# georgeliu233/STrajNet

Hardware: AMD Instinct MI355X
Metric: scenes/sec (fwd+bwd, 256x256 grids) (higher is better)
Workload: dtype bf16; 1 GPU; STrajNet cfg-256 train step (fwd+OGMFlow_loss+bwd+Nadam), batch 8/GPU, 8 waypoints, obs+occ+flow heads, fg_msa+fg, random-init weights; global_batch=8, grid=256x256x11, parallelism=dp1, hipgraph=True, concurrent_branch_streams=True, optimizer_in_step=True, settle_steps=40

## Files before the change

### include/strajnet_hip.h

```cpp
#ifndef STRAJNET_HIP_H
#define STRAJNET_HIP_H
#include <hip/hip_runtime_api.h>
#ifdef __cplusplus
extern "C" {
#endif

enum stj_status { STJ_OK = 0, STJ_EINVAL = -1, STJ_ELAUNCH = -2, STJ_EUNSUPPORTED = -3 };
enum stj_dtype { STJ_F32 = 0, STJ_BF16 = 1, STJ_F16 = 2 };
enum stj_act { STJ_ACT_NONE = 0, STJ_ACT_GELU = 1, STJ_ACT_ELU = 2 };
enum stj_unary { STJ_U_GELU = 1, STJ_U_ELU = 2, STJ_U_TANH_SCALE = 3 };

const char* stj_last_error(void);
int stj_abi_version(void);

int stj_gemm(const void* A, const void* B, void* C, const float* bias, const void* res, float* colsum,
             int M, int N, int K, int nb1, int nb2,
             long long sAb1, long long sAb2, long long sAm, long long sAk,
             long long sBb1, long long sBb2, long long sBk, long long sBn,
             long long sCb1, long long sCb2, long long ldc,
             long long sBias1, long long sBias2, long long sRes1, long long sRes2, long long ldres,
             int act, float alpha, int dtype, int c_f32, int accumulate, int splitk,
             int nkb, long long sAkb, long long sBkb, void* group, hipStream_t stream);
long long stj_gemm_group_workspace_bytes(void);
int stj_gemm_group_begin(void* group);
// ... 174 lines not shown
                       int Wi, int Cin, int Cout, int dtype, hipStream_t stream);
int stj_elu_res_bwd(const void* dy, const void* dy2, const void* y, const void* r, void* dpre, void* gsum, long long n, int dtype,
                    hipStream_t stream);
int stj_skip_junction_bwd(const void* dy1, const void* dy2, const void* y, const void* r1, const void* r2, void* dpre, void* dr1,
                          void* dr2, long long n, int dtype, hipStream_t stream);
int stj_upconv_dgrad(const void* dP, const void* Wd, void* dX, const void* Xelu, int F, int Hi, int Wi, int Cin, int Cout,
                     int dtype, hipStream_t stream);
int stj_upconv_wgrad(const void* X, const void* dP, float* dWeff, float* dbias, int db_parts, int F, int Hi, int Wi, int Cin,
                     int Cout, int wg_budget, int dtype, hipStream_t stream);
int stj_outconv_fwd(const void* X, const float* W, const float* bias, float* Y, int F, int Hh, int Ww, int C, int Tn,
                    long long y_bstride, long long y_tstride, long long y_pstride, int dtype, hipStream_t stream);
int stj_outconv_pair_fwd(const void* X0, const void* X1, const float* W0, const float* W1, const float* bias0, const float* bias1,
                         float* Y, int B, int Tn, int H, int W, int C, int t_major, int dtype, hipStream_t stream);
int stj_upconv_fwd_head(const void* X, const void* Wf, const float* bias, const float* Whead, void* Z, int F, int Hi, int Wi, int Cin,
                        int Cout, int dtype, hipStream_t stream);
int stj_outconv_pair_gather(const void* Z0, const void* Z1, const float* bias0, const float* bias1, float* Y, int B, int Tn, int H, int W,
                            int t_major, int dtype, hipStream_t stream);
int stj_quantize_waypoints(const float* Y, uint8_t* Q, int B, int Tn, int H, int W, hipStream_t stream);
int stj_outconv_pair_gather_q(const void* Z0, const void* Z1, const float* bias0, const float* bias1, uint8_t* Q, int B, int Tn, int H,
                              int W, int t_major, int dtype, hipStream_t stream);
int stj_compress_sizes(int B, int Tn, int H, int W, long long* work_bytes, long long* out_capacity);
int stj_compress_waypoints(const uint8_t* Q, void* work, uint8_t* out, uint32_t* offsets, int B, int Tn, int H, int W, hipStream_t stream);
int stj_outconv_bwd(const void* X, const float* W, const float* dY, void* dX, float* dW, float* db, int F, int Hh, int Ww,
                    int C, int Tn, long long y_bstride, long long y_tstride, long long y_pstride, int elu_in, void* ws,
                    long long ws_bytes, int dtype, hipStream_t stream);
long long stj_outconv_bwd_workspace_bytes(void);
int stj_im2col_patch(const float* src, void* dst, int B, int H, int W, int Cin, long long pix_stride, int ch_stride,
                     int dtype, hipStream_t stream);
int stj_patch_embed_supported(int Cin, int Cout, int dtype);
int stj_patch_embed_fwd(const float* src, const void* w, const float* bias, const float* gamma, const float* beta, const void* add,
                        const float* gamma2, const float* beta2, void* cols, void* pre, void* x2, void* y, float* mean, float* rstd,
                        float* mean2, float* rstd2, int B, int H, int W, int Cin, long long pix_stride, int ch_stride, int Cout,
                        float eps, int dtype, hipStream_t stream);
int stj_im2col3(const void* x, void* cols, int N, int H, int W, int G, int Cg, int dtype, hipStream_t stream);
int stj_col2im3(const void* dcols, void* dx, int N, int H, int W, int G, int Cg, int dtype, hipStream_t stream);

int stj_loss_auc_gate(const float* gt_obs, const float* gt_occ, const float* gt_flow, const float* origin,
                      int* hist, float* gate, float* auc_out, int B, int H, int W, hipStream_t stream);
int stj_loss_fwd(const float* logits, const float* gt_obs, const float* gt_occ, const float* gt_flow, const float* origin,
                 const float* gate, float* sums, float* loss, float* coef, int B, int H, int W, float ogm_w, float occ_w,
                 float flow_origin_w, float replica, int flags, hipStream_t stream);
int stj_loss_bwd(const float* logits, const float* gt_obs, const float* gt_occ, const float* gt_flow, const float* origin,
                 const float* coef, const float* upstream, float* dlogits, int B, int H, int W, int flags, hipStream_t stream);
int stj_loss_coef(const float* gt_flow, const float* gate, int* cnt, float* coef, int B, int H, int W, float ogm_w, float occ_w,
                  float flow_origin_w, float replica, int flags, hipStream_t stream);
int stj_loss_finalize(const float* sums, const float* gate, float* loss, float* coef_out, int B, int H, int W, float ogm_w,
                      float occ_w, float flow_origin_w, float replica, int flags, hipStream_t stream);
int stj_loss_gate_coef(const float* gt_obs, const float* gt_occ, const float* gt_flow, const float* origin, int* hist, float* gate,
                       float* auc_out, float* coef, int B, int H, int W, float ogm_w, float occ_w, float flow_origin_w,
                       float replica, int flags, hipStream_t stream);
int stj_loss_fwd_bwd(const float* logits, const float* gt_obs, const float* gt_occ, const float* gt_flow, const float* origin,
                     const float* gate, const float* coef_in, float* sums, float* loss, float* coef_out, float* dlogits,
                     int B, int H, int W, float ogm_w, float occ_w, float flow_origin_w, float replica, int flags, hipStream_t stream);

int stj_decode_raw(const void* src, int kind, float* dst, long long n_outer, int H, int W, int C, int y0, int x0, int Ho,
                   int Wo, float scale, hipStream_t stream);

int stj_unpack_bits(const uint32_t* bits, float* dst, long long n_total, hipStream_t stream);
int stj_unpack_sparse(const uint32_t* mask, const uint32_t* offs, const uint32_t* val_base, const float* vals, long long n_vals,
                      float* dst, int B, long long n, hipStream_t stream);

int stj_agent_prep(const float* obs, const float* occ, int n_obs, int n_occ, int B, int Tn, void* x5, void* v3, int* vt, int* cmi,
                   void* cmf, int dtype, hipStream_t stream);
int stj_agent_mix_fwd(const void* enc, const void* embed, const void* cm, void* concat, void* qin, int B, int A, int C, int dtype,
                      hipStream_t stream);
int stj_agent_mix_bwd(const void* dconcat, const void* dqin, const void* cm, void* denc, void* dembed, int B, int A, int C, int dtype,
// ... 35 lines not shown
```

### strajnet_amd/build.py

```python
import os
import subprocess
import sys
from concurrent.futures import ThreadPoolExecutor

HERE = os.path.dirname(os.path.abspath(__file__))
CSRC = os.path.join(HERE, 'csrc')
OUT = os.path.join(HERE, 'libstrajnet_hip.so')
HEADER = os.path.join(os.path.dirname(HERE), 'include', 'strajnet_hip.h')
SOURCES = ['util.hip', 'gemm.hip', 'wgrad_sk.hip', 'norm.hip', 'patch_embed.hip', 'swin_attn.hip', 'swin_fused.hip', 'xattn_fused.hip', 'fgattn.hip', 'agent_fused.hip', 'fgoff_fused.hip', 'attn.hip', 'conv.hip', 'conv_ws.hip', 'conv_ps.hip', 'loss.hip', 'eval.hip', 'quantize.hip', 'deflate.hip', 'unpack.hip', 'rng.hip']
FLAGS = ['--offload-arch=gfx950', '-O3', '-std=c++17', '-fPIC', '-munsafe-fp-atomics', '-Wno-unused-result', '-Wno-unused-value',
         '-ffp-contract=fast']


def _hipcc():
    for c in (os.environ.get('HIPCC'), '/opt/rocm/bin/hipcc', 'hipcc'):
        if c and (os.path.sep not in c or os.path.exists(c)):
            return c
    raise RuntimeError('hipcc not found')


def _stale(target, deps):
    if not os.path.exists(target):
        return True
    t = os.path.getmtime(target)
    return any(os.path.getmtime(d) > t for d in deps)


def build(force=False, verbose=True):
    hipcc = _hipcc()
    hdrs = [HEADER] + [os.path.join(CSRC, f) for f in os.listdir(CSRC) if f.endswith('.h')]
    objs, jobs = [], []
    os.makedirs(os.path.join(HERE, 'build'), exist_ok=True)
    for s in SOURCES:
        src = os.path.join(CSRC, s)
        obj = os.path.join(HERE, 'build', s.replace('.hip', '.o'))
        objs.append(obj)
        if force or _stale(obj, [src] + hdrs):
            jobs.append([hipcc] + FLAGS + ['-c', src, '-o', obj])

    def run(cmd):
        r = subprocess.run(cmd, capture_output=True, text=True)
        return cmd, r
# ... 17 lines not shown
```

### strajnet_amd/modules.py

```python
import math
import os
from collections import OrderedDict

import numpy as np
import torch

from . import ops
from .ops import Param, ACT_NONE, ACT_ELU


def _param_spec(cfg, hb, fg_msa, fg):
    C, ws, heads, depths = cfg['embed_dim'], cfg['window_size'], cfg['num_heads'], cfg['depths']
    sp = OrderedDict()

    def add(name, shape, init):
        assert name not in sp
        sp[name] = (tuple(shape), init)

    def dense(n, i, o, bias=True):
        add(n + '/kernel', (i, o), 'glorot')
        if bias:
            add(n + '/bias', (o,), 'zeros')

    def conv(n, kh, kw, i, o, bias=True):
# ... 153 lines not shown
        self._zstride = offs['cross_attn_obs1/norm1/gamma'] - offs['cross_attn_obs0/norm1/gamma']
        for n in spec:
            if n.startswith('cross_attn_obs0/'):
                for z in range(1, 8):
                    assert offs[n.replace('obs0', f'obs{z}')] - offs[n] == z * self._zstride
        self._flat = torch.zeros(off, dtype=torch.float32, device=self.device)
        self._goff8 = (off + ops._ZeroArena.ALIGN - 1) // ops._ZeroArena.ALIGN * ops._ZeroArena.ALIGN
        self._gbuf = torch.zeros(self._goff8 + ops._ZeroArena.FLOATS, dtype=torch.float32, device=self.device)
        self._gflat = self._gbuf[:off]
        self._cflat = self._flat if dtype == torch.float32 else torch.zeros(off, dtype=dtype, device=self.device)
        gen = torch.Generator().manual_seed(seed)
        dpr = np.linspace(0.0, 0.1, sum(cfg['depths']))
        self.drop_path_rate = {}
        for i, d in enumerate(cfg['depths']):
            for j in range(d):
                self.drop_path_rate[f'layers{i}/blocks{j}'] = float(dpr[sum(cfg['depths'][:i]) + j])
        for j in range(cfg['depths'][0]):
            self.drop_path_rate[f'flow_layers0/blocks{j}'] = float(dpr[j])
        self._seg_onehot = {}
        self.dropctx = ops.DropCtx(self.device, seed if dropout_seed is None else dropout_seed)
        self._arena = ops._ZeroArena()
        self._arena.adopt(self._gbuf[self._goff8:])
        self._dctx = None
        self._side = ops.role_stream(self.device, 'side') if (self.device.type == 'cuda' and os.environ.get('STJ_NO_SIDE_STREAM') != '1') else None
        self._side2 = ops.role_stream(self.device, 'side2') if (self._side is not None and os.environ.get('STJ_NO_SIDE_STREAM') != '2') else None
        self._streams = (self._side, self._side2)
        self.serial = False
        self.taps = None
        self.fused_mlp = self.fused_attn = os.environ.get('STJ_FUSED_SWIN', '1') != '0'
        self.fused_attn_dims = (96, 192, 384)
        self.fused_mlp_dims = (96, 192, 384)
        self.fused_xattn = True
        self.fused_stem = True
        self.agent_override = None
        self._quantize_heads = False
        self.mid_forward_hook = None
        self.fused_fgattn = True
        self.fused_agent = True
        self.fused_agent_int = True
        self.fused_quantize = True
        self.fused_fgoff = True
        self._agent_pack = None
        self._agent_pack_event = None
        self._agent_pack_stale = True
        self._fgoff_pack = None
        self._fgoff_pack_event = None
        self._fgoff_pack_stale = True
        self._xattn_pack = None
        self.params = OrderedDict()
        for n, (s, kind) in spec.items():
            k = int(np.prod(s))
            sl = slice(offs[n], offs[n] + k)
            self._flat[sl] = _init_tensor(s, kind, gen).reshape(-1).to(self.device)
            master = self._flat[sl].view(s).requires_grad_(True)
            grad = self._gflat[sl].view(s)
            master.grad = grad
            self.params[n] = Param(n, s, master, self._cflat[sl].view(s), grad)
        def wants_parts(n):
            leaf = n.rsplit('/', 1)[-1]
            if n.startswith('cross_attn_obs'):
                return False
            return leaf in ('gamma', 'beta', 'relative_position_bias_table') or (leaf == 'bias' and '/upconv' in n)
        names = [n for n in spec if wants_parts(n)]
        P = self.PARTS
        self._parts = torch.zeros(P * sum(int(np.prod(spec[n][0])) for n in names), dtype=torch.float32, device=self.device)
        idx, o = [], 0
# ... 120 lines not shown
        qkv = self._dense(h, pre + '/attn/qkv')
        a = ops.win_attn(qkv, self._p(pre + '/attn/relative_position_bias_table'), B, res, heads, shift)

        def mlp_fused(x):
            return ops.swin_mlp(x, self._p(pre + '/norm2/gamma'), self._p(pre + '/norm2/beta'), self._p(pre + '/mlp/fc1/kernel'),
                                self._p(pre + '/mlp/fc1/bias'), self._p(pre + '/mlp/fc2/kernel'), self._p(pre + '/mlp/fc2/bias'), 1e-5,
                                self._dctx, pre + '/drop_path_mlp', dpr, rows_per_sample=res * res)
        if dpr == 0.0:
            x = self._dense(a, pre + '/attn/proj', res=x)
            if fused_mlp:
                return mlp_fused(x)
            h, x = self._ln_skip(x, pre + '/norm2', 1e-5)
            h = ops.gelu(self._dense(h, pre + '/mlp/fc1'))
            return self._dense(h, pre + '/mlp/fc2', res=x)
        a = self._dense(a, pre + '/attn/proj').view(B, -1)
        x = ops.dropout(a, dpr, self._dctx, pre + '/drop_path_attn', res=x.view(B, -1), per_sample=True).view(x.shape)
        if fused_mlp:
            return mlp_fused(x)
        h, x = self._ln_skip(x, pre + '/norm2', 1e-5)
        h = ops.gelu(self._dense(h, pre + '/mlp/fc1'))
        h = self._dense(h, pre + '/mlp/fc2').view(B, -1)
        return ops.dropout(h, dpr, self._dctx, pre + '/drop_path_mlp', res=x.view(B, -1), per_sample=True).view(x.shape)

    def _tap(self, name, t):
        if self.taps is not None:
            self.taps[name] = t.detach().float().clone()

    def _basic_layer(self, x, pre, B, res, depth, heads, downsample, add=None):
        for i in range(depth):
            x = self._swin_block(x, f'{pre}/blocks{i}', B, res, heads, 0 if i % 2 == 0 else 4)
            self._tap(f'{pre}/block{i}', x)
        if not downsample:
            return x, x
        m = self._ln(x, pre + '/downsample/norm', 1e-5, gather_res=res)
        if callable(add):
            add = add()
        return self._dense(m, pre + '/downsample/reduction', bias=False, res=add), x

    def _patch_embed(self, src, name, Cin, ch_stride, pix_stride, add=None, norm2=None):
        B, H = src.shape[0], src.shape[1]
        pw = self._p(name + '/proj/kernel')
        if self.fused_stem and ops.patch_embed_ok(Cin, pw.c.shape[-1], self.dtype):
            y = ops.patch_embed(src, pw, self._p(name + '/proj/bias'), self._p(name + '/norm/gamma'), self._p(name + '/norm/beta'),
                                Cin, ch_stride, pix_stride, self.dtype, 1e-5, add,
                                self._p(norm2 + '/gamma') if norm2 else None, self._p(norm2 + '/beta') if norm2 else None)
            return y.view(B, (H // 4) ** 2, -1)
        cols = ops.patch_im2col(src, Cin, ch_stride, pix_stride, self.dtype)
        y = self._dense(cols, name + '/proj')
        y = self._ln(y, name + '/norm', 1e-5, res=add.view(y.shape) if add is not None else None)
        if norm2:
            y = self._ln(y, norm2, 1e-5)
        return y.view(B, (H // 4) ** 2, -1)

    def _encoder(self, ogm, map_img, flow, hook=None):
        B = ogm.shape[0]
        C, P = self.stage_dim[0], self.P
        depths, heads = self.cfg['depths'], self.cfg['num_heads']
        def flow_branch():
            fl = self._patch_embed(flow, 'patch_embed_flow', 2, 1, 2, norm2='flow_norm')
            return self._basic_layer(fl, 'flow_layers0', B, P, depths[0], heads[0], True)
        side = self._side2
        if side is not None:
            main = torch.cuda.current_stream(self.device)
            side.wait_stream(main)
            with torch.cuda.stream(side):
                flow_x, flow_res = flow_branch()
# ... 441 lines not shown
```

### strajnet_amd/ops.py

```python
import contextlib
import ctypes

import os
import threading

import torch

from . import prof
from ._lib import call as _raw_call, ENUMS as _ENUMS


def call(name, *args):
    if prof.ACTIVE is None:
        return _raw_call(name, *args)
    prof.record(name, args, lambda: _raw_call(name, *args))


GROUP_GEMMS = os.environ.get('STJ_GEMM_GROUP', '1') != '0'
WS_KERNELS = os.environ.get('STJ_NO_WS') != '1'
class _GroupState(threading.local):
    def __init__(self):
        self.h = [None, None]
        self.depth = [0]

# ... 1770 lines not shown
        cols, pre, x2, mean, rstd, mean2, rstd2 = ctx.saved_tensors
        gw, pbias, pg, pb, pg2, pb2 = ctx.p
        M, N = pre.shape
        K = cols.shape[1]
        dy = dy.contiguous().view(M, N)
        if pg2 is not None and LN_CHAIN and _ln_chain_ok(N, dy.dtype):
            dpre = torch.empty_like(pre)
            d2 = torch.empty_like(pre) if ctx.has_add else None
            (g2, b2, n2, s2), (g1, b1, n1, s1) = _ln_grad_targets(pg2, pb2), _ln_grad_targets(pg, pb)
            call('stj_layernorm_bwd_chain', _p(dy), _p(x2), _p(pg2.master), _p(mean2), _p(rstd2), _p(pre), _p(pg.master), _p(mean), _p(rstd),
                 _p(d2), _p(dpre), _p(g2), _p(b2), _p(g1), _p(b1), M, N, n2, s2, n1, s1, _dt(pre), _st())
            dadd = d2.view(ctx.add_shape) if ctx.has_add else None
        else:
            if pg2 is not None:
                dy = _ln_bwd_plain(dy, x2, mean2, rstd2, pg2, pb2, M, N)
            dadd = dy.view(ctx.add_shape) if ctx.has_add else None
            dpre = _ln_bwd_plain(dy, pre, mean, rstd, pg, pb, M, N)
        gemm(cols, dpre, gw, K, N, M, (0, 0, 1, K), (0, 0, N, 1), (0, 0, N), _dt(cols), c_f32=1, accumulate=1, splitk=0,
             colsum=pbias.grad)
        return (None,) * 7 + (dadd,) + (None,) * 4


def patch_embed_ok(Cin, Cout, dtype):
    from ._lib import lib
    return bool(lib().stj_patch_embed_supported(Cin, Cout, DTYPE_CODE[dtype]))


def patch_embed(src, pw, pbias, pg, pb, Cin, ch_stride, pix_stride, dtype, eps=1e-5, add=None, pg2=None, pb2=None):
    N = pw.c.shape[-1]
    return _PatchEmbed.apply(src, pw.master, pw.c.view(-1, N), pw.grad.view(-1, N), pbias, pg, pb, add, pg2, pb2,
                             (Cin, ch_stride, pix_stride, eps, torch.is_grad_enabled()), dtype)


def patch_im2col(src, Cin, ch_stride, pix_stride, dtype):
    _req_cuda(src)
    src = src.contiguous()
    B, H, W = src.shape[0], src.shape[1], src.shape[2]
    out = torch.empty((B * (H // 4) * (W // 4), 16 * Cin), dtype=dtype, device=src.device)
    call('stj_im2col_patch', _p(src), _p(out), B, H, W, Cin, pix_stride, ch_stride, DTYPE_CODE[dtype], _st())
    return out


class _GroupedConv3(torch.autograd.Function):
    @staticmethod
    def forward(ctx, x, w_master, b_master, pw, pb, G):
        _req_cuda(x)
        x = x.contiguous()
        N, H, W, C = x.shape
        Cg = C // G
        K = 9 * Cg
        Co = pw.c.shape[-1]
        cog = Co // G
        dt = _dt(x)
        M = N * H * W
        cols = torch.empty((M, G, K), dtype=x.dtype, device=x.device)
        call('stj_im2col3', _p(x), _p(cols), N, H, W, G, Cg, dt, _st())
        y = torch.empty((N, H, W, Co), dtype=x.dtype, device=x.device)
        gemm(cols, pw.c, y, M, cog, K, (0, K, G * K, 1), (0, cog, Co, 1), (0, cog, Co), dt, bias=pb.master, sBias=(0, cog), nb=(1, G))
        ctx.pw, ctx.pb, ctx.geo = pw, pb, (N, H, W, G, Cg, K, Co, cog, M)
        ctx.save_for_backward(cols)
        return y

    @staticmethod
    def backward(ctx, dy):
        (cols,) = ctx.saved_tensors
        N, H, W, G, Cg, K, Co, cog, M = ctx.geo
# ... 423 lines not shown
```

### strajnet_amd/prof.py

```python
import torch

ACTIVE = None
COST = {}


def enable():
    global ACTIVE
    ACTIVE = {}


def disable():
    global ACTIVE
    p, ACTIVE = ACTIVE, None
    return p


def _es(dt):
    return 4 if dt == 0 else 2


def _gemm(a):
    (M, N, K, nb1, nb2) = a[6:11]
    sAb1, sAb2, sAm, sAk, sBb1, sBb2, sBk, sBn = a[11:19]
    act, alpha, dt, c_f32, acc, splitk, nkb = a[27], a[28], a[29], a[30], a[31], a[32], a[33]
# ... 126 lines not shown


def _elem(fam, n_idx, dt_idx, tensors, f32=False):
    def f(a):
        n = a[n_idx]
        es = 4 if f32 else _es(a[dt_idx])
        return f'{fam}[{n}]', fam, 0.0, 0.0, tensors * es * n
    return f


def _loss(fam, tens):
    def f(a):
        B, H, W = (a[9], a[10], a[11]) if fam == 'loss_fwd' else ((a[11], a[12], a[13]) if fam == 'loss_fwd_bwd' else (a[8], a[9], a[10]))
        by = 4.0 * B * H * W * (32 * tens + 8 * 5)
        return f'{fam}[B{B} {H}x{W}]', fam, 0.0, 0.0, by
    return f


def _eval(a):
    B, H, W = a[11], a[12], a[13]
    return f'eval_fwd[B{B} {H}x{W}]', 'eval_fwd', 0.0, 0.0, 4.0 * B * H * W * (32 + 8 * 5)


def _patch_embed(a):
    B, H, W, Cin, pix, Cout, dt = a[16], a[17], a[18], a[19], a[20], a[22], a[24]
    es = _es(dt)
    M = B * (H // 4) * (W // 4)
    nz = lambda i: bool(getattr(a[i], 'value', None))
    by = 4.0 * B * H * W * pix + es * M * Cout * (1 + nz(5) + nz(9) + nz(10)) + es * M * 16 * Cin * nz(8)
    fl = 2.0 * M * 16 * Cin * Cout
    return f'patch_embed[{H}x{W},{Cin}->{Cout},B{B}]', 'patch_embed_fwd', fl, fl, by


def _ln_chain(a):
    rows, C, dt = a[15], a[16], a[21]
    return f'ln_bwd_chain[{rows}x{C}]', 'layernorm_bwd', 0.0, 0.0, _es(dt) * rows * C * (4 + bool(getattr(a[9], 'value', None)))


MODELS = {
    'stj_gemm': _gemm,
    'stj_patch_embed_fwd': _patch_embed, 'stj_layernorm_bwd_chain': _ln_chain,
    'stj_upconv_fwd': _upconv('fwd'), 'stj_upconv_fwd_head': _upconv_head, 'stj_outconv_pair_gather': _pair_gather, 'stj_outconv_pair_gather_q': _pair_gather_q, 'stj_quantize_waypoints': _quantize, 'stj_compress_waypoints': _compress, 'stj_upconv_fwd_res': _upconv_res, 'stj_elu_res_bwd': _elu_res, 'stj_upconv_dgrad': _upconv('dgrad'), 'stj_upconv_wgrad': _upconv('wgrad'),
    'stj_outconv_fwd': _outconv('fwd'), 'stj_outconv_pair_fwd': _outconv_pair, 'stj_outconv_bwd': _outconv('bwd'),
    'stj_layernorm_fwd': _ln('fwd'), 'stj_layernorm_bwd': _ln('bwd'), 'stj_layernorm_res_fwd': _ln('res_fwd'),
    'stj_win_attn_fwd': _win('fwd'), 'stj_win_attn_bwd': _win('bwd'),
    'stj_unary_fwd': _elem('unary_fwd', 2, 5, 2), 'stj_unary_bwd': _elem('unary_bwd', 3, 6, 3),
    'stj_dropout': _elem('dropout', 3, 8, 2),
    'stj_loss_fwd': _loss('loss_fwd', 1), 'stj_loss_bwd': _loss('loss_bwd', 2), 'stj_loss_fwd_bwd': _loss('loss_fwd_bwd', 2),
    'stj_eval_fwd': _eval,
    'stj_nadam_step': _elem('nadam', 4, 0, 7, f32=True),
}
EXTRA_MODELS = {}


def record(name, args, launch):
    m = MODELS.get(name) or EXTRA_MODELS.get(name)
    if m is not None:
        try:
            key, fam, fa, fe, by = m(args)
        except Exception:
            key, fam, fa, fe, by = name, name.replace('stj_', ''), 0.0, 0.0, 0.0
    else:
        key, fam, fa, fe, by = name, name.replace('stj_', ''), 0.0, 0.0, 0.0
    st = torch.cuda.current_stream()
    e0, e1 = torch.cuda.Event(enable_timing=True), torch.cuda.Event(enable_timing=True)
    e0.record(st)
    launch()
    e1.record(st)
    COST[key] = (fam, fa, fe, by)
    ACTIVE.setdefault(key, []).append((e0, e1))


def summarize(events, steps):
    keys = {}
# ... 15 lines not shown
```

Baseline: 1415 scenes/s.

## Fuse Swin patch-merge gather, LayerNorm and reduction GEMM into one kernel

Adds a patch-merge forward kernel that gathers the 2x2 neighbourhood, applies LayerNorm in registers and runs the reduction matmul from LDS with MFMA, adding the optional residual in the epilogue. A matching backward kernel computes the dgrad GEMM, the LayerNorm backward, the skip-gradient add and the dgamma/dbeta partials, then scatters dx back into the original layout. The goal is to avoid the separate gathered LayerNorm output round trip and several launches at the stage-1/2 downsamples. The weight-grad GEMM stays separate, and the normalized activations are still stored for it when grad is on.

```diff
diff --git a/include/strajnet_hip.h b/include/strajnet_hip.h
--- a/include/strajnet_hip.h
+++ b/include/strajnet_hip.h
@@ -230,6 +230,12 @@
                         const float* gamma2, const float* beta2, void* cols, void* pre, void* x2, void* y, float* mean, float* rstd,
                         float* mean2, float* rstd2, int B, int H, int W, int Cin, long long pix_stride, int ch_stride, int Cout,
                         float eps, int dtype, hipStream_t stream);
+int stj_patch_merge_supported(int C0, int dtype);
+int stj_patch_merge_fwd(const void* x, const float* gamma, const float* beta, const void* w, const void* add, void* y, void* m,
+                        float* mean, float* rstd, int B, int res, int C0, float eps, int dtype, hipStream_t stream);
+int stj_patch_merge_bwd(const void* dy, const void* w, const void* x, const float* gamma, const float* mean, const float* rstd,
+                        const void* dskip, void* dx, float* dgamma, float* dbeta, int B, int res, int C0, int nparts,
+                        long long part_stride, int dtype, hipStream_t stream);
 int stj_im2col3(const void* x, void* cols, int N, int H, int W, int G, int Cg, int dtype, hipStream_t stream);
 int stj_col2im3(const void* dcols, void* dx, int N, int H, int W, int G, int Cg, int dtype, hipStream_t stream);
 
diff --git a/strajnet_amd/build.py b/strajnet_amd/build.py
--- a/strajnet_amd/build.py
+++ b/strajnet_amd/build.py
@@ -7,7 +7,7 @@
 CSRC = os.path.join(HERE, 'csrc')
 OUT = os.path.join(HERE, 'libstrajnet_hip.so')
 HEADER = os.path.join(os.path.dirname(HERE), 'include', 'strajnet_hip.h')
-SOURCES = ['util.hip', 'gemm.hip', 'wgrad_sk.hip', 'norm.hip', 'patch_embed.hip', 'swin_attn.hip', 'swin_fused.hip', 'xattn_fused.hip', 'fgattn.hip', 'agent_fused.hip', 'fgoff_fused.hip', 'attn.hip', 'conv.hip', 'conv_ws.hip', 'conv_ps.hip', 'loss.hip', 'eval.hip', 'quantize.hip', 'deflate.hip', 'unpack.hip', 'rng.hip']
+SOURCES = ['util.hip', 'gemm.hip', 'wgrad_sk.hip', 'norm.hip', 'patch_embed.hip', 'patch_merge.hip', 'swin_attn.hip', 'swin_fused.hip', 'xattn_fused.hip', 'fgattn.hip', 'agent_fused.hip', 'fgoff_fused.hip', 'attn.hip', 'conv.hip', 'conv_ws.hip', 'conv_ps.hip', 'loss.hip', 'eval.hip', 'quantize.hip', 'deflate.hip', 'unpack.hip', 'rng.hip']
 FLAGS = ['--offload-arch=gfx950', '-O3', '-std=c++17', '-fPIC', '-munsafe-fp-atomics', '-Wno-unused-result', '-Wno-unused-value',
          '-ffp-contract=fast']
 
diff --git a/strajnet_amd/csrc/patch_merge.hip b/strajnet_amd/csrc/patch_merge.hip
--- /dev/null
+++ b/strajnet_amd/csrc/patch_merge.hip
@@ -0,0 +1,434 @@
+#include "common.h"
+
+namespace pm {
+
+constexpr int RB = 32;
+constexpr int VN = 8;
+typedef __attribute__((ext_vector_type(4))) uint32_t u32x4;
+
+template <int C0>
+__device__ __forceinline__ size_t src_off(unsigned row, int c, int res) {
+  const unsigned half = (unsigned)res >> 1;
+  const unsigned j = row % half, t = row / half, i = t % half, b = t / half;
+  const int q = c / C0, cc = c - q * C0;
+  return (((size_t)b * res + 2 * i + (q & 1)) * res + 2 * j + (q >> 1)) * C0 + cc;
+}
+template <typename T> __device__ __forceinline__ void unpack8(const uint4& u, float* v) {
+  unpack2<T>(u.x, v[0], v[1]); unpack2<T>(u.y, v[2], v[3]); unpack2<T>(u.z, v[4], v[5]); unpack2<T>(u.w, v[6], v[7]);
+}
+template <typename T> __device__ __forceinline__ uint4 pack8(const float* v) {
+  return make_uint4(pack2<T>(v[0], v[1]), pack2<T>(v[2], v[3]), pack2<T>(v[4], v[5]), pack2<T>(v[6], v[7]));
+}
+
+template <typename T, int WN, int CPR, int N>
+__device__ __forceinline__ void fwd_load_w(u32x4 (&wv)[WN], const T* w, int tid) {
+#pragma unroll
+  for (int j = 0; j < WN; ++j) {
+    const int p = tid + 256 * j, k = p / CPR, c = (p % CPR) * VN;
+    wv[j] = *reinterpret_cast<const u32x4*>(w + (size_t)k * N + c);
+  }
+}
+
+template <typename T, int WN, int CPR, int LDW>
+__device__ __forceinline__ void fwd_stage_w(T* Ws, const u32x4 (&wv)[WN], int tid) {
+  __syncthreads();
+#pragma unroll
+  for (int j = 0; j < WN; ++j) {
+    const int p = tid + 256 * j, k = p / CPR, c = (p % CPR) * VN;
+    *reinterpret_cast<u32x4*>(Ws + k * LDW + c) = wv[j];
+  }
+  __syncthreads();
+}
+template <typename T, int NF, int KC, int LDA, int LDW>
+__device__ __forceinline__ void fwd_mma_chunk(const T* As, const T* Ws, int k0, int rh, int ch, int lane, f32x4 (&acc)[NF]) {
+#pragma unroll
+  for (int kk = 0; kk < KC; kk += 32) {
+    const typename Mma<T>::Frag tok = Mma<T>::load(As, LDA, 16 * rh, k0 + kk, lane);
+#pragma unroll
+    for (int n = 0; n < NF; ++n) acc[n] = Mma<T>::mma(Mma<T>::load_tr(Ws, LDW, (ch * NF + n) * 16, kk, lane), tok, acc[n]);
+  }
+}
+
+struct FwdArgs {
+  const void* x; const float* gamma; const float* beta; const void* w; const void* add;
+  void* y; void* m; float* mean; float* rstd;
+  long long rows; int res; float eps;
+};
+
+template <typename T, int C0, int NF>
+struct FwdGeo {
+  static constexpr int K = 4 * C0, N = 2 * C0, NS = 32 * NF;
+  static constexpr int KC = 12288 / NS;
+  static constexpr int LDA = K + LdsPad<T>::P;
+  static constexpr int LDW = NS + 16;
+  static constexpr size_t lds_bytes = (size_t)(RB * LDA + KC * LDW) * sizeof(T);
+  static_assert(K % KC == 0 && N % NS == 0 && KC % 32 == 0, "whole chunks and slices");
+};
+
+template <typename T, int C0, int NF>
+__global__ __launch_bounds__(256) void patch_merge_fwd_kernel(FwdArgs a) {
+  typedef FwdGeo<T, C0, NF> G;
+  constexpr int K = G::K, N = G::N, NS = G::NS, KC = G::KC, LDA = G::LDA, LDW = G::LDW;
+  constexpr int CPR = NS / VN, WN = KC * CPR / 256;
+  constexpr int NCHK = (K / VN + 63) / 64, RPW = RB / 4;
+  static_assert(KC * CPR % 256 == 0, "whole pieces per thread");
+  extern __shared__ __attribute__((aligned(16))) unsigned char smem[];
+  T* As = reinterpret_cast<T*>(smem);
+  T* Ws = As + RB * LDA;
+  const int tid = threadIdx.x, lane = tid & 63, wave = tid >> 6;
+  const long long m0 = (long long)blockIdx.x * RB;
+  const int n0 = blockIdx.y * NS;
+  const T* w = reinterpret_cast<const T*>(a.w) + n0;
+
+  constexpr int NCH = K / KC;
+  u32x4 wa[WN], wb[WN];
+  fwd_load_w<T, WN, CPR, N>(wa, w, tid);
+  if (NCH > 1) fwd_load_w<T, WN, CPR, N>(wb, w + (size_t)KC * N, tid);
+
+  {
+    const T* x = reinterpret_cast<const T*>(a.x);
+    uint4 raw[RPW][NCHK];
+#pragma unroll
+    for (int u = 0; u < RPW; ++u) {
+      const long long row = min(m0 + wave * RPW + u, a.rows - 1);
+#pragma unroll
+      for (int k = 0; k < NCHK; ++k) {
+        const int c = min((lane + 64 * k) * VN, K - VN);
+        raw[u][k] = *reinterpret_cast<const uint4*>(x + src_off<C0>((unsigned)row, c, a.res));
+      }
+    }
+    float gam[NCHK][VN], bet[NCHK][VN];
+#pragma unroll
+    for (int k = 0; k < NCHK; ++k) {
+      const int c = min((lane + 64 * k) * VN, K - VN);
+#pragma unroll
+      for (int e = 0; e < VN; e += 4) {
+        const float4 gv = *reinterpret_cast<const float4*>(a.gamma + c + e), bv = *reinterpret_cast<const float4*>(a.beta + c + e);
+        gam[k][e] = gv.x; gam[k][e + 1] = gv.y; gam[k][e + 2] = gv.z; gam[k][e + 3] = gv.w;
+        bet[k][e] = bv.x; bet[k][e + 1] = bv.y; bet[k][e + 2] = bv.z; bet[k][e + 3] = bv.w;
+      }
+    }
+    constexpr float invC = 1.f / K;
+#pragma unroll
+    for (int u = 0; u < RPW; ++u) {
+      const int r = wave * RPW + u;
+      const bool ok = m0 + r < a.rows;
+      float v[NCHK][VN];
+      float s = 0.f;
+#pragma unroll
+      for (int k = 0; k < NCHK; ++k) {
+        const bool in = (lane + 64 * k) * VN < K;
+        unpack8<T>(raw[u][k], v[k]);
+#pragma unroll
+        for (int e = 0; e < VN; ++e) { v[k][e] = in ? v[k][e] : 0.f; s += v[k][e]; }
+      }
+      const float mu = wave_sum(s) * invC;
+      float q = 0.f;
+#pragma unroll
+      for (int k = 0; k < NCHK; ++k) {
+        const bool in = (lane + 64 * k) * VN < K;
+#pragma unroll
+        for (int e = 0; e < VN; ++e) { const float d = in ? v[k][e] - mu : 0.f; q += d * d; }
+      }
+      const float rs = rsqrtf(wave_sum(q) * invC + a.eps);
+#pragma unroll
+      for (int k = 0; k < NCHK; ++k) {
+        const int c = (lane + 64 * k) * VN;
+        if (c >= K) continue;
+        float o[VN];
+#pragma unroll
+        for (int e = 0; e < VN; ++e) o[e] = ok ? (v[k][e] - mu) * rs * gam[k][e] + bet[k][e] : 0.f;
+        const uint4 pk = pack8<T>(o);
+        *reinterpret_cast<uint4*>(As + r * LDA + c) = pk;
+        if (a.m && ok && blockIdx.y == 0) *reinterpret_cast<uint4*>(reinterpret_cast<T*>(a.m) + (m0 + r) * K + c) = pk;
+      }
+      if (a.mean && ok && blockIdx.y == 0 && lane == 0) { a.mean[m0 + r] = mu; a.rstd[m0 + r] = rs; }
+    }
+  }
+
+  const int rh = wave & 1, ch = wave >> 1, g = lane >> 4;
+  const long long mrow = m0 + 16 * rh + (lane & 15);
+  uint2 addv[NF];
+  {
+    const T* ad = reinterpret_cast<const T*>(a.add ? a.add : a.y) + min(mrow, a.rows - 1) * N + n0 + ch * NF * 16 + 4 * g;
+#pragma unroll
+    for (int n = 0; n < NF; ++n) addv[n] = *reinterpret_cast<const uint2*>(ad + n * 16);
+  }
+  f32x4 acc[NF];
+#pragma unroll
+  for (int n = 0; n < NF; ++n) acc[n] = (f32x4){0.f, 0.f, 0.f, 0.f};
+#pragma unroll 1
+  for (int kc = 0; kc < NCH; kc += 2) {
+    fwd_stage_w<T, WN, CPR, LDW>(Ws, wa, tid);
+    if (kc + 2 < NCH) fwd_load_w<T, WN, CPR, N>(wa, w + (size_t)(kc + 2) * KC * N, tid);
+    fwd_mma_chunk<T, NF, KC, LDA, LDW>(As, Ws, kc * KC, rh, ch, lane, acc);
+    if (kc + 1 < NCH) {
+      fwd_stage_w<T, WN, CPR, LDW>(Ws, wb, tid);
+      if (kc + 3 < NCH) fwd_load_w<T, WN, CPR, N>(wb, w + (size_t)(kc + 3) * KC * N, tid);
+      fwd_mma_chunk<T, NF, KC, LDA, LDW>(As, Ws, (kc + 1) * KC, rh, ch, lane, acc);
+    }
+  }
+
+  if (mrow < a.rows) {
+    const bool has_add = a.add != nullptr;
+#pragma unroll
+    for (int n = 0; n < NF; ++n) {
+      float v[4] = {acc[n][0], acc[n][1], acc[n][2], acc[n][3]}, r[4];
+      unpack2<T>(addv[n].x, r[0], r[1]); unpack2<T>(addv[n].y, r[2], r[3]);
+#pragma unroll
+      for (int e = 0; e < 4; ++e) v[e] += has_add ? r[e] : 0.f;
+      st4(reinterpret_cast<T*>(a.y) + mrow * N + n0 + (ch * NF + n) * 16 + 4 * g, v);
+    }
+  }
+}
+
+struct BwdArgs {
+  const void* dy; const void* w; const void* x; const float* gamma; const float* mean; const float* rstd; const void* dskip;
+  void* dx; float* dgamma; float* dbeta;
+  long long rows; int res; int nparts; long long pstride;
+};
+
+template <typename T, int C0>
+struct BwdGeo {
+  static constexpr int K = 4 * C0, N = 2 * C0;
+  static constexpr int LDD = N + LdsPad<T>::P, LDM = K + LdsPad<T>::P;
+  static constexpr size_t lds_bytes = (size_t)(RB * LDD + RB * LDM) * sizeof(T);
+  static_assert(8 * 2 * K * sizeof(float) <= lds_bytes, "the waves' dgamma / dbeta partials reuse the two tiles");
+};
+
+template <typename T, int C0>
+__global__ __launch_bounds__(512) void patch_merge_bwd_kernel(BwdArgs a) {
+  typedef BwdGeo<T, C0> G;
+  constexpr int K = G::K, N = G::N, LDD = G::LDD, LDM = G::LDM;
+  constexpr int NW = 8, NST = N / 32, IT = K / 16 / NW;
+  constexpr int NCHK = (K / VN + 63) / 64, RPW = RB / NW;
+  static_assert(K % (16 * NW) == 0 && N % 32 == 0, "whole row groups per wave");
+  extern __shared__ __attribute__((aligned(16))) unsigned char smem[];
+  T* Ds = reinterpret_cast<T*>(smem);
+  T* Dm = Ds + RB * LDD;
+  const int tid = threadIdx.x, lane = tid & 63, wave = tid >> 6, g = lane >> 4;
+  const long long m0 = (long long)blockIdx.x * RB;
+  const T* w = reinterpret_cast<const T*>(a.w);
+
+  typename Mma<T>::Frag wf[NST];
+  auto load_w = [&](int kg) {
+#pragma unroll
+    for (int ns = 0; ns < NST; ++ns) wf[ns] = Mma<T>::from_global(w + (size_t)(kg * 16 + (lane & 15)) * N + ns * 32 + 8 * g);
+  };
+  load_w(wave);
+
+  {
+    constexpr int CPR = N / VN, PER = (RB * CPR + 511) / 512;
+    const T* dy = reinterpret_cast<const T*>(a.dy);
+    uint4 v[PER];
+#pragma unroll
+    for (int j = 0; j < PER; ++j) {
+      const int p = min(tid + 512 * j, RB * CPR - 1), r = p / CPR, c = (p % CPR) * VN;
+      v[j] = *reinterpret_cast<const uint4*>(dy + min(m0 + r, a.rows - 1) * N + c);
+    }
+#pragma unroll
+    for (int j = 0; j < PER; ++j) {
+      const int p = tid + 512 * j, r = p / CPR, c = (p % CPR) * VN;
+      if (p < RB * CPR) *reinterpret_cast<uint4*>(Ds + r * LDD + c) = m0 + r < a.rows ? v[j] : make_uint4(0, 0, 0, 0);
+    }
+  }
+  uint4 xr[RPW][NCHK], sr[RPW][NCHK];
+  float mu[RPW], rs[RPW];
+  {
+    const T* x = reinterpret_cast<const T*>(a.x);
+    const T* ds = reinterpret_cast<const T*>(a.dskip ? a.dskip : a.x);
+    const bool has_skip = a.dskip != nullptr;
+#pragma unroll
+    for (int u = 0; u < RPW; ++u) {
+      const long long row = min(m0 + wave * RPW + u, a.rows - 1);
+      mu[u] = a.mean[row]; rs[u] = a.rstd[row];
+#pragma unroll
+      for (int k = 0; k < NCHK; ++k) {
+        const size_t off = src_off<C0>((unsigned)row, min((lane + 64 * k) * VN, K - VN), a.res);
+        xr[u][k] = *reinterpret_cast<const uint4*>(x + off);
+        sr[u][k] = *reinterpret_cast<const uint4*>(ds + off);
+        if (!has_skip) sr[u][k] = make_uint4(0, 0, 0, 0);
+      }
+    }
+  }
+  float gam[NCHK][VN];
+#pragma unroll
+  for (int k = 0; k < NCHK; ++k) {
+    const int c = min((lane + 64 * k) * VN, K - VN);
+#pragma unroll
+    for (int e = 0; e < VN; e += 4) {
+      const float4 gv = *reinterpret_cast<const float4*>(a.gamma + c + e);
+      gam[k][e] = gv.x; gam[k][e + 1] = gv.y; gam[k][e + 2] = gv.z; gam[k][e + 3] = gv.w;
+    }
+  }
+  __syncthreads();
+
+#pragma unroll 1
+  for (int it = 0; it < IT; ++it) {
+    const int kg = wave + NW * it;
+    typename Mma<T>::Frag cur[NST];
+#pragma unroll
+    for (int ns = 0; ns < NST; ++ns) cur[ns] = wf[ns];
+    if (it + 1 < IT) load_w(kg + NW);
+    f32x4 acc[2] = {(f32x4){0.f, 0.f, 0.f, 0.f}, (f32x4){0.f, 0.f, 0.f, 0.f}};
+#pragma unroll
+    for (int ns = 0; ns < NST; ++ns) {
+#pragma unroll
+      for (int rh = 0; rh < 2; ++rh) acc[rh] = Mma<T>::mma(cur[ns], Mma<T>::load(Ds, LDD, 16 * rh, 32 * ns, lane), acc[rh]);
+    }
+#pragma unroll
+    for (int rh = 0; rh < 2; ++rh) {
+      const float v[4] = {acc[rh][0], acc[rh][1], acc[rh][2], acc[rh][3]};
+      st4(Dm + (16 * rh + (lane & 15)) * LDM + kg * 16 + 4 * g, v);
+    }
+  }
+  __syncthreads();
+
+  {
+    constexpr float invC = 1.f / K;
+    float ag[NCHK][VN], ab[NCHK][VN];
+#pragma unroll
+    for (int k = 0; k < NCHK; ++k)
+#pragma unroll
+      for (int e = 0; e < VN; ++e) { ag[k][e] = 0.f; ab[k][e] = 0.f; }
+    T* dx = reinterpret_cast<T*>(a.dx);
+#pragma unroll
+    for (int u = 0; u < RPW; ++u) {
+      const int r = wave * RPW + u;
+      const bool ok = m0 + r < a.rows;
+      float dv[NCHK][VN], xv[NCHK][VN];
+      float s1 = 0.f, s2 = 0.f;
+#pragma unroll
+      for (int k = 0; k < NCHK; ++k) {
+        const int c = (lane + 64 * k) * VN;
+        const bool in = ok && c < K;
+        unpack8<T>(*reinterpret_cast<const uint4*>(Dm + r * LDM + min(c, K - VN)), dv[k]);
+        unpack8<T>(xr[u][k], xv[k]);
+#pragma unroll
+        for (int e = 0; e < VN; ++e) {
+          const float d = in ? dv[k][e] : 0.f;
+          const float xh = in ? (xv[k][e] - mu[u]) * rs[u] : 0.f;
+          const float gg = d * gam[k][e];
+          ag[k][e] += d * xh;
+          ab[k][e] += d;
+          xv[k][e] = xh; dv[k][e] = gg;
+          s1 += gg; s2 += gg * xh;
+        }
+      }
+      s1 = wave_sum(s1) * invC;
+      s2 = wave_sum(s2) * invC;
+      if (!ok) continue;
+#pragma unroll
+      for (int k = 0; k < NCHK; ++k) {
+        const int c = (lane + 64 * k) * VN;
+        if (c >= K) continue;
+        float o[VN], sk[VN];
+        unpack8<T>(sr[u][k], sk);
+#pragma unroll
+        for (int e = 0; e < VN; ++e) o[e] = rs[u] * (dv[k][e] - s1 - xv[k][e] * s2) + sk[e];
+        *reinterpret_cast<uint4*>(dx + src_off<C0>((unsigned)(m0 + r), c, a.res)) = pack8<T>(o);
+      }
+    }
+    __syncthreads();
+    float* part = reinterpret_cast<float*>(smem);
+#pragma unroll
+    for (int k = 0; k < NCHK; ++k) {
+      const int c = (lane + 64 * k) * VN;
+      if (c >= K) continue;
+#pragma unroll
+      for (int e = 0; e < VN; e += 4) {
+        *reinterpret_cast<float4*>(part + (wave * 2 + 0) * K + c + e) = make_float4(ag[k][e], ag[k][e + 1], ag[k][e + 2], ag[k][e + 3]);
+        *reinterpret_cast<float4*>(part + (wave * 2 + 1) * K + c + e) = make_float4(ab[k][e], ab[k][e + 1], ab[k][e + 2], ab[k][e + 3]);
+      }
+    }
+  }
+  __syncthreads();
+  const float* part = reinterpret_cast<const float*>(smem);
+  const long long po = (long long)(blockIdx.x % a.nparts) * a.pstride;
+  for (int c = tid; c < 2 * K; c += 512) {
+    float sum = 0.f;
+#pragma unroll
+    for (int wv = 0; wv < NW; ++wv) sum += part[wv * 2 * K + c];
+    atomicAdd((c < K ? a.dgamma + c : a.dbeta + (c - K)) + po, sum);
+  }
+}
+
+template <typename T, int C0, int NF>
+static int launch_fwd(const FwdArgs& a, hipStream_t stream) {
+  typedef FwdGeo<T, C0, NF> G;
+  if (!stj_reserve_lds<patch_merge_fwd_kernel<T, C0, NF>>((int)G::lds_bytes)) {
+    stj_set_error("stj_patch_merge_fwd: cannot reserve %zu bytes of LDS", G::lds_bytes);
+    return STJ_ELAUNCH;
+  }
+  const dim3 grid((unsigned)((a.rows + RB - 1) / RB), G::N / G::NS);
+  hipLaunchKernelGGL((patch_merge_fwd_kernel<T, C0, NF>), grid, dim3(256), G::lds_bytes, stream, a);
+  return stj_check_launch("stj_patch_merge_fwd");
+}
+template <typename T, int C0>
+static int fwd_by_slices(const FwdArgs& a, hipStream_t stream) {
+  const long long blocks = (a.rows + RB - 1) / RB * (2 * C0 / 192);
+  return blocks >= 192 ? launch_fwd<T, C0, 6>(a, stream) : launch_fwd<T, C0, 3>(a, stream);
+}
+template <typename T, int C0>
+static int launch_bwd(const BwdArgs& a, hipStream_t stream) {
+  typedef BwdGeo<T, C0> G;
+  if (!stj_reserve_lds<patch_merge_bwd_kernel<T, C0>>((int)G::lds_bytes)) {
+    stj_set_error("stj_patch_merge_bwd: cannot reserve %zu bytes of LDS", G::lds_bytes);
+    return STJ_ELAUNCH;
+  }
+  hipLaunchKernelGGL((patch_merge_bwd_kernel<T, C0>), dim3((unsigned)((a.rows + RB - 1) / RB)), dim3(512), G::lds_bytes, stream, a);
+  return stj_check_launch("stj_patch_merge_bwd");
+}
+
+static int check_geo(const char* entry, int B, int res, int C0, int dtype, long long* rows) {
+  if (!stj_dtype_ok(dtype)) { stj_set_error("%s: bad dtype %d", entry, dtype); return STJ_EINVAL; }
+  if (!stj_patch_merge_supported(C0, dtype)) {
+    stj_set_error("%s: C0 %d / dtype %d not built (C0 in {96, 192}, 16-bit storage types)", entry, C0, dtype);
+    return STJ_EUNSUPPORTED;
+  }
+  if (B <= 0 || res <= 0 || (res & 1)) { stj_set_error("%s: bad geometry (B %d, res %d: res must be even)", entry, B, res); return STJ_EINVAL; }
+  *rows = (long long)B * (res / 2) * (res / 2);
+  if (*rows >= (1ll << 31)) { stj_set_error("%s: %lld rows (32-bit row arithmetic inside the kernel)", entry, *rows); return STJ_EUNSUPPORTED; }
+  return STJ_OK;
+}
+
+}
+
+extern "C" int stj_patch_merge_supported(int C0, int dtype) { return (C0 == 96 || C0 == 192) && stj_is16(dtype); }
+
+extern "C" int stj_patch_merge_fwd(const void* x, const float* gamma, const float* beta, const void* w, const void* add, void* y, void* m,
+                                   float* mean, float* rstd, int B, int res, int C0, float eps, int dtype, hipStream_t stream) {
+  long long rows = 0;
+  if (const int rc = pm::check_geo("stj_patch_merge_fwd", B, res, C0, dtype, &rows)) return rc;
+  if (!x || !gamma || !beta || !w || !y || (!m) != (!mean) || (!m) != (!rstd) ||
+      (((uintptr_t)x | (uintptr_t)gamma | (uintptr_t)beta | (uintptr_t)w | (uintptr_t)add | (uintptr_t)y | (uintptr_t)m) & 15)) {
+    stj_set_error("stj_patch_merge_fwd: bad arguments (null / unaligned pointer; m, mean and rstd come together)");
+    return STJ_EINVAL;
+  }
+  pm::FwdArgs a{x, gamma, beta, w, add, y, m, mean, rstd, rows, res, eps};
+  int r = STJ_EUNSUPPORTED;
+  stj_with_dtype16(dtype, [&](auto t) {
+    typedef typename decltype(t)::type T;
+    r = C0 == 96 ? pm::fwd_by_slices<T, 96>(a, stream) : pm::fwd_by_slices<T, 192>(a, stream);
+  });
+  return r;
+}
+
+extern "C" int stj_patch_merge_bwd(const void* dy, const void* w, const void* x, const float* gamma, const float* mean, const float* rstd,
+                                   const void* dskip, void* dx, float* dgamma, float* dbeta, int B, int res, int C0, int nparts,
+                                   long long part_stride, int dtype, hipStream_t stream) {
+  long long rows = 0;
+  if (const int rc = pm::check_geo("stj_patch_merge_bwd", B, res, C0, dtype, &rows)) return rc;
+  if (!dy || !w || !x || !gamma || !mean || !rstd || !dx || !dgamma || !dbeta || nparts < 1 || (nparts > 1 && part_stride < 4 * C0) ||
+      (((uintptr_t)dy | (uintptr_t)w | (uintptr_t)x | (uintptr_t)dskip | (uintptr_t)dx) & 15)) {
+    stj_set_error("stj_patch_merge_bwd: bad arguments (null / unaligned pointer, nparts / part_stride)");
+    return STJ_EINVAL;
+  }
+  pm::BwdArgs a{dy, w, x, gamma, mean, rstd, dskip, dx, dgamma, dbeta, rows, res, nparts, part_stride};
+  int r = STJ_EUNSUPPORTED;
+  stj_with_dtype16(dtype, [&](auto t) {
+    typedef typename decltype(t)::type T;
+    r = C0 == 96 ? pm::launch_bwd<T, 96>(a, stream) : pm::launch_bwd<T, 192>(a, stream);
+  });
+  return r;
+}
diff --git a/strajnet_amd/modules.py b/strajnet_amd/modules.py
--- a/strajnet_amd/modules.py
+++ b/strajnet_amd/modules.py
@@ -209,6 +209,7 @@
         self.fused_mlp_dims = (96, 192, 384)
         self.fused_xattn = True
         self.fused_stem = True
+        self.fused_merge = True
         self.agent_override = None
         self._quantize_heads = False
         self.mid_forward_hook = None
@@ -395,6 +396,11 @@
             self._tap(f'{pre}/block{i}', x)
         if not downsample:
             return x, x
+        if self.fused_merge and ops.patch_merge_ok(x.shape[-1], self.dtype):
+            if callable(add):
+                add = add()
+            return ops.patch_merge(x, self._p(pre + '/downsample/norm/gamma'), self._p(pre + '/downsample/norm/beta'),
+                                   self._p(pre + '/downsample/reduction/kernel'), 1e-5, res, add)
         m = self._ln(x, pre + '/downsample/norm', 1e-5, gather_res=res)
         if callable(add):
             add = add()
diff --git a/strajnet_amd/ops.py b/strajnet_amd/ops.py
--- a/strajnet_amd/ops.py
+++ b/strajnet_amd/ops.py
@@ -1826,6 +1826,62 @@
                              (Cin, ch_stride, pix_stride, eps, torch.is_grad_enabled()), dtype)
 
 
+class _PatchMerge(torch.autograd.Function):
+    @staticmethod
+    def forward(ctx, x, trig, wc, gw, pg, pb, add, geo):
+        _req_cuda(x)
+        eps, gres, grad_on = geo
+        x = x.contiguous()
+        B, L, C0 = x.shape
+        assert L == gres * gres
+        K, N = wc.shape
+        assert K == 4 * C0 and N == 2 * C0
+        rows = B * (gres // 2) ** 2
+        dev = x.device
+        y = torch.empty((B, (gres // 2) ** 2, N), dtype=x.dtype, device=dev)
+        m = mean = rstd = None
+        if grad_on:
+            m = torch.empty((rows, K), dtype=x.dtype, device=dev)
+            mean, rstd = torch.empty(rows, dtype=torch.float32, device=dev), torch.empty(rows, dtype=torch.float32, device=dev)
+        a2 = add.contiguous().view(rows, N) if add is not None else None
+        call('stj_patch_merge_fwd', _p(x), _p(pg.master), _p(pb.master), _p(wc), _p(a2), _p(y), _p(m), _p(mean), _p(rstd), B, gres, C0,
+             float(eps), _dt(x), _st())
+        ctx.p = (wc, gw, pg, pb)
+        ctx.geo = (B, gres, C0)
+        ctx.has_add, ctx.add_shape = add is not None, (add.shape if add is not None else None)
+        ctx.save_for_backward(x, m, mean, rstd)
+        return y, x.view_as(x)
+
+    @staticmethod
+    def backward(ctx, dy, dskip=None):
+        x, m, mean, rstd = ctx.saved_tensors
+        if dy is None:
+            return (dskip,) + (None,) * 7
+        wc, gw, pg, pb = ctx.p
+        B, gres, C0 = ctx.geo
+        K, N = wc.shape
+        rows = m.shape[0]
+        dt = _dt(x)
+        dy2 = dy.contiguous().view(rows, N)
+        dx = torch.empty_like(x)
+        dres = dskip.contiguous() if dskip is not None else None
+        dg, db, nparts, pstride = _ln_grad_targets(pg, pb)
+        call('stj_patch_merge_bwd', _p(dy2), _p(wc), _p(x), _p(pg.master), _p(mean), _p(rstd), _p(dres), _p(dx), _p(dg), _p(db), B, gres, C0,
+             nparts, pstride, dt, _st())
+        gemm(m, dy2, gw, K, N, rows, (0, 0, 1, K), (0, 0, N, 1), (0, 0, N), dt, c_f32=1, accumulate=1, splitk=0)
+        return dx, None, None, None, None, None, (dy.view(ctx.add_shape) if ctx.has_add else None), None
+
+
+def patch_merge_ok(C0, dtype):
+    from ._lib import lib
+    return bool(lib().stj_patch_merge_supported(C0, DTYPE_CODE[dtype]))
+
+
+def patch_merge(x, pg, pb, pw, eps, gather_res, add=None):
+    N = pw.c.shape[-1]
+    return _PatchMerge.apply(x, pw.master, pw.c.view(-1, N), pw.grad.view(-1, N), pg, pb, add, (eps, gather_res, torch.is_grad_enabled()))
+
+
 def patch_im2col(src, Cin, ch_stride, pix_stride, dtype):
     _req_cuda(src)
     src = src.contiguous()
diff --git a/strajnet_amd/prof.py b/strajnet_amd/prof.py
--- a/strajnet_amd/prof.py
+++ b/strajnet_amd/prof.py
@@ -182,6 +182,22 @@
     return f'patch_embed[{H}x{W},{Cin}->{Cout},B{B}]', 'patch_embed_fwd', fl, fl, by
 
 
+def _patch_merge(kind):
+    def f(a):
+        nz = lambda i: bool(getattr(a[i], 'value', None))
+        if kind == 'fwd':
+            B, res, C0, dt = a[9], a[10], a[11], a[13]
+            rows, K, N = B * (res // 2) ** 2, 4 * C0, 2 * C0
+            by = _es(dt) * (rows * K * (1 + nz(6)) + rows * N * (1 + nz(4)) + K * N)
+        else:
+            B, res, C0, dt = a[10], a[11], a[12], a[15]
+            rows, K, N = B * (res // 2) ** 2, 4 * C0, 2 * C0
+            by = _es(dt) * (rows * K * (2 + nz(6)) + rows * N + K * N)
+        fl = 2.0 * rows * K * N
+        return f'patch_merge_{kind}[{rows}x{K}->{N}]', 'patch_merge_' + kind, fl, fl, by
+    return f
+
+
 def _ln_chain(a):
     rows, C, dt = a[15], a[16], a[21]
     return f'ln_bwd_chain[{rows}x{C}]', 'layernorm_bwd', 0.0, 0.0, _es(dt) * rows * C * (4 + bool(getattr(a[9], 'value', None)))
@@ -190,6 +206,7 @@
 MODELS = {
     'stj_gemm': _gemm,
     'stj_patch_embed_fwd': _patch_embed, 'stj_layernorm_bwd_chain': _ln_chain,
+    'stj_patch_merge_fwd': _patch_merge('fwd'), 'stj_patch_merge_bwd': _patch_merge('bwd'),
     'stj_upconv_fwd': _upconv('fwd'), 'stj_upconv_fwd_head': _upconv_head, 'stj_outconv_pair_gather': _pair_gather, 'stj_outconv_pair_gather_q': _pair_gather_q, 'stj_quantize_waypoints': _quantize, 'stj_compress_waypoints': _compress, 'stj_upconv_fwd_res': _upconv_res, 'stj_elu_res_bwd': _elu_res, 'stj_upconv_dgrad': _upconv('dgrad'), 'stj_upconv_wgrad': _upconv('wgrad'),
     'stj_outconv_fwd': _outconv('fwd'), 'stj_outconv_pair_fwd': _outconv_pair, 'stj_outconv_bwd': _outconv('bwd'),
     'stj_layernorm_fwd': _ln('fwd'), 'stj_layernorm_bwd': _ln('bwd'), 'stj_layernorm_res_fwd': _ln('res_fwd'),
```

Measured after the change: 1422 scenes/s (median of 6 runs). About the same (+0.5%).
